# facebookresearch/iris

Measured on AMD Instinct MI355X. Metric: bake_shading throughput (shading samples/s: secondary rays traced and shaded), higher is better.
Workload: dtype f32; 1 GPU; bake_shading train-view sequence (15 views evenly spaced among 32 cameras on a circle, one view per step), 1920x1080, SPP=128 per lobe, lobes=[0, 1, 2, 3, 4, 5, 6] (0=diffuse,1-6=specular), synthetic room seed=1 1000990 triangles, SLF H=256, Philox uniforms; pixels_per_view=2073600

## Files before the change

### iris_amd/_lib.py

```python
import ctypes as C
import os

import torch

_HERE = os.path.dirname(os.path.abspath(__file__))
LIB_PATH = os.environ.get("IRIS_HIP_LIB") or os.path.join(_HERE, "libiris_hip.so")

BVH_DEFAULT, BVH4_F32, BVH4_Q8 = 0, 1, 3
BAKE_AUTO, BAKE_PIXEL_PER_WAVE, BAKE_TILE_SORTED = 0, 1, 2


class IrisError(RuntimeError):
    pass


class SceneInfo(C.Structure):
    _fields_ = [("n_vertices", C.c_int64), ("n_triangles", C.c_int64), ("layout", C.c_int32), ("n_nodes", C.c_int32),
                ("node_bytes", C.c_int32), ("tri_bytes", C.c_int32), ("depth", C.c_int32), ("n_leaf_records", C.c_int32),
                ("sah_cost", C.c_float), ("build_seconds", C.c_float)]


_P, _I64, _I32, _F, _D, _U64, _U32 = C.c_void_p, C.c_int64, C.c_int, C.c_float, C.c_double, C.c_uint64, C.c_uint32


# ... 143 lines not shown
    "iris_version": [],
}
_RESTYPE = {"iris_scene_destroy": None, "iris_slf_destroy": None, "iris_emitter_destroy": None,
            "iris_last_error": C.c_char_p, "iris_version": C.c_char_p, "iris_debug_build_flags": C.c_char_p, "iris_debug_source_hash": C.c_char_p, "iris_ngp_n_params": C.c_int64, "iris_ngp_destroy": None, "iris_bake_workspace_bytes": C.c_uint64, "iris_pt_compact_workspace_bytes": C.c_uint64, "iris_denoise_workspace_bytes": C.c_uint64,
            "iris_exr_zip_workspace_bytes": C.c_uint64, "iris_ngp_backward_workspace_bytes": C.c_uint64, "iris_crf_bwd_workspace_bytes": C.c_uint64,
            "iris_loss_photometric_workspace_bytes": C.c_uint64,
            "iris_png_row_bytes": C.c_int64, "iris_png_stream_bound": C.c_uint64, "iris_png_workspace_bytes": C.c_uint64, "iris_png_magma_table": None,
            "iris_jpeg_stream_bound": C.c_uint64, "iris_jpeg_workspace_bytes": C.c_uint64, "iris_jpeg_tables": None,
            "iris_image_metrics_workspace_bytes": C.c_uint64, "iris_uv_raster_workspace_bytes": C.c_uint64, "iris_atlas_density": C.c_double}

_lib = None


def lib():
    global _lib
    if _lib is None:
        if not os.path.exists(LIB_PATH):
            raise IrisError(f"{LIB_PATH} is missing: build it with `make -C iris_amd/csrc` or "
                            "`python -c 'import __graft_entry__ as g; g.build()'`. There is no CPU fallback.")
        l = C.CDLL(LIB_PATH)
        for name, argtypes in PROTOTYPES.items():
            fn = getattr(l, name)
            fn.argtypes = argtypes
            fn.restype = _RESTYPE.get(name, C.c_int)
        _lib = l
    return _lib


def source_hash():
    import hashlib
    h = hashlib.sha256()
    h.update(lib().iris_debug_build_flags())
    root = os.path.dirname(_HERE)
    files = [os.path.join("iris_amd", "csrc", f) for f in ("bvh_build.cpp", "bvh_build.h", "iris_bake.h", "iris_device.h", "iris_hip.hip", "iris_tile.h", "iris_trace.h")]
    files += [os.path.join("include", "iris_hip.h"), os.path.join("include", "iris_hip_debug.h")]
    for f in files:
        h.update(f.encode()); h.update(open(os.path.join(root, f), "rb").read())
    return h.hexdigest()[:16]


def device_index(device):
    device = torch.device(device)
    if device.type != "cuda":
        raise IrisError(f"{device}: the HIP path needs a GPU device (there is no CPU fallback)")
    return device.index if device.index is not None else torch.cuda.current_device()


class Native:

    def __init__(self, ptr=None, destroy=None, device=None, keys=()):
        self.ptr, self.destroy, self.device, self.keys = ptr, destroy, device, list(keys)

    def free(self):
        d = self.__dict__
        p, d["ptr"] = d.get("ptr"), None
        if p:
            d["destroy"](p)

    def __del__(self):
        try:
            self.free()
        except Exception:
            pass

    def __reduce__(self):
        return (Native, ())

# ... 93 lines not shown
```

### iris_amd/csrc/iris_bake.h

```cpp
#pragma once
#include "iris_tile.h"

namespace iris {

struct BakeArgs {
    SceneDev sc; EmitDev em; SlfDev slf;
    const float* pos; const float* nrm; const float* wo;
    const float* u2; const int32_t* pix_id;
    int64_t P; int spp; uint64_t seed; uint32_t stream_id; float rough;
    float* out0; float* out1; int64_t* tri_next;
    int64_t* src_next;
    unsigned long long* stats;
    uint32_t* stack_ovf;
    float4* scratch;
    unsigned int* tile_counter;
    int tile_px;
};

#ifndef IRIS_TILE_RAYS
#define IRIS_TILE_RAYS 5120
#endif
constexpr int kTileRays = IRIS_TILE_RAYS;

__device__ __forceinline__ void reduce_geometry(int spp, int& lpp, int& ppw, int& rounds) {
// ... 219 lines not shown
                    const f3 pn = hit_position(h, mk3(tx.x, ty.x, tz.x), mk3(tx.y, ty.y, tz.y), mk3(tx.z, ty.z, tz.z));
                    q = make_float4(pn.x, pn.y, pn.z, ow);
                }
                res[r] = q;
            } else
            res[r] = make_float4(h.u, h.v, __int_as_float(h.slot), 0.f);
            if (COUNT) n_rays++; }
        );

    const int n_groups = (np + ppw - 1) / ppw;
    IRIS_PHASE_BEGIN();
    for (int g = wave; g < n_groups; g += kBlock / 64) {
        const int pl = g * ppw + sub;
        const bool pvalid = pl < np;
        float a0x = 0.f, a0y = 0.f, a0z = 0.f, a1x = 0.f, a1y = 0.f, a1z = 0.f;
        if (resolve) {
            for (int rr = 0; rr < rounds; rr += 2) {
                const int s0 = rr * 64 + sl, s1 = s0 + 64;
                const bool ok0 = pvalid && s0 < spp, ok1 = pvalid && rr + 1 < rounds && s1 < spp;
                float4 q0 = make_float4(0.f, 0.f, 0.f, __int_as_float(-2)), q1 = q0;
                float2 w0 = make_float2(0.f, 0.f), w1 = w0;
                if (ok0) { q0 = res[pl * spp + s0]; if (SPEC) w0 = res_g[pl * spp + s0]; }
                if (ok1) { q1 = res[pl * spp + s1]; if (SPEC) w1 = res_g[pl * spp + s1]; }
                const int o0 = __float_as_int(q0.w), o1 = __float_as_int(q1.w);
                int j0 = -1, j1 = -1;
                if (o0 == -1) j0 = slf_index(a.slf, mk3(q0.x, q0.y, q0.z));
                if (o1 == -1) j1 = slf_index(a.slf, mk3(q1.x, q1.y, q1.z));
                float4 r0 = make_float4(0.f, 0.f, 0.f, 0.f), r1 = r0;
                if (o0 >= 0 || j0 >= 0) r0 = *(o0 >= 0 ? a.em.radiance + o0 : a.slf.radiance + j0);
                if (o1 >= 0 || j1 >= 0) r1 = *(o1 >= 0 ? a.em.radiance + o1 : a.slf.radiance + j1);
                if (ok0) {
                    const float z = o0 >= 0 ? -0.f : 0.f;
                    const f3 Le = mk3(z + r0.x, z + r0.y, z + r0.z);
                    if (a.src_next) a.src_next[(p0 + pl) * spp + s0] = o0 >= 0 ? -2 - o0 : j0;
                    if (SPEC) { a0x += Le.x * w0.y; a0y += Le.y * w0.y; a0z += Le.z * w0.y; a1x += Le.x * w0.x; a1y += Le.y * w0.x; a1z += Le.z * w0.x; }
                    else { a0x += Le.x; a0y += Le.y; a0z += Le.z; }
                }
                if (ok1) {
                    const float z = o1 >= 0 ? -0.f : 0.f;
                    const f3 Le = mk3(z + r1.x, z + r1.y, z + r1.z);
                    if (a.src_next) a.src_next[(p0 + pl) * spp + s1] = o1 >= 0 ? -2 - o1 : j1;
                    if (SPEC) { a0x += Le.x * w1.y; a0y += Le.y * w1.y; a0z += Le.z * w1.y; a1x += Le.x * w1.x; a1y += Le.y * w1.x; a1z += Le.z * w1.x; }
                    else { a0x += Le.x; a0y += Le.y; a0z += Le.z; }
                }
            }
        } else
        for (int rr = 0; rr < rounds; ++rr) {
            const int s = rr * 64 + sl;
            if (pvalid && s < spp) {
                const float4 qa = res[pl * spp + s];
                Hit h; h.u = qa.x; h.v = qa.y; h.slot = __float_as_int(qa.z); h.t = 0.f; h.id = 0;
                f3 pn = mk3(0.f, 0.f, 0.f);
                int64_t tri = -1;
                int ord_rec = -1;
                if (h.slot >= 0) {
                    const float4* tr = a.sc.tris + (int64_t)h.slot * 4;
                    const float4 tx = tr[0], ty = tr[1], tz = tr[2];
                    if (!a.em.emit_ord) ord_rec = __float_as_int(tr[3].x);
                    pn = hit_position(h, mk3(tx.x, ty.x, tz.x), mk3(tx.y, ty.y, tz.y), mk3(tx.z, ty.z, tz.z));
                    tri = __float_as_int(tx.w);
                }
                if (a.tri_next) a.tri_next[(p0 + pl) * spp + s] = tri;
                float epdf; bool vn; int src;
                const f3 Le = eval_emitter1(a.em, a.slf, pn, tri, true, 1.0f, 0.0f, epdf, vn, src, ord_rec);
                if (a.src_next) a.src_next[(p0 + pl) * spp + s] = src;
                if (SPEC) {
                    const float2 qb = res_g[pl * spp + s];
                    a0x += Le.x * qb.y; a0y += Le.y * qb.y; a0z += Le.z * qb.y;
                    a1x += Le.x * qb.x; a1y += Le.y * qb.x; a1z += Le.z * qb.x;
                } else { a0x += Le.x; a0y += Le.y; a0z += Le.z; }
            }
        }
        for (int m = 1; m < lpp; m <<= 1) {
            a0x += __shfl_xor(a0x, m); a0y += __shfl_xor(a0y, m); a0z += __shfl_xor(a0z, m);
// ... 100 lines not shown
```

### iris_amd/csrc/iris_device.h

```cpp
#pragma once
#include <hip/hip_runtime.h>
#include <stdint.h>

namespace iris {

struct f3 { float x, y, z; };
__device__ __forceinline__ f3 mk3(float x, float y, float z) { f3 r; r.x = x; r.y = y; r.z = z; return r; }
__device__ __forceinline__ f3 ld3(const float* p) { return mk3(p[0], p[1], p[2]); }
__device__ __forceinline__ void st3(float* p, f3 a) { p[0] = a.x; p[1] = a.y; p[2] = a.z; }
__device__ __forceinline__ f3 sub3(f3 a, f3 b) { return mk3(a.x - b.x, a.y - b.y, a.z - b.z); }

__device__ __forceinline__ f3 x_cross(f3 a, f3 b) {
    return mk3(fmaf(a.y, b.z, -(a.z * b.y)), fmaf(a.z, b.x, -(a.x * b.z)), fmaf(a.x, b.y, -(a.y * b.x)));
}
__device__ __forceinline__ float x_dot(f3 a, f3 b) { return fmaf(a.z, b.z, fmaf(a.y, b.y, a.x * b.x)); }

__device__ __forceinline__ float t_dot(f3 a, f3 b) { return (a.x * b.x + a.y * b.y) + a.z * b.z; }
__device__ __forceinline__ f3 t_normalize(f3 a) {
    float n = sqrtf((a.x * a.x + a.y * a.y) + a.z * a.z);
    n = fmaxf(n, 1e-12f);
    return mk3(a.x / n, a.y / n, a.z / n);
}
__device__ __forceinline__ f3 t_cross(f3 a, f3 b) {
    return mk3(a.y * b.z - a.z * b.y, a.z * b.x - a.x * b.z, a.x * b.y - a.y * b.x);
}
__device__ __forceinline__ float relu(float x) { return x > 0.f ? x : 0.f; }

constexpr float kPi = 3.14159265358979323846f;
constexpr float kTwoPi = 6.28318530717958647692f;
constexpr float kRayEps = 8.940696716308594e-05f;

__device__ __forceinline__ void normal_space(f3 n, f3& t, f3& b) {
    if (fabsf(n.x) <= 0.1f) t = t_normalize(mk3(0.f, -n.z, n.y));
    else                    t = t_normalize(mk3(n.z, 0.f, -n.x));
    b = t_cross(n, t);
// ... 104 lines not shown
    return r;
}

__device__ __forceinline__ void philox_u2(uint64_t seed, uint64_t idx, uint32_t stream, float& u0, float& u1) {
    uint32_t c0 = (uint32_t)idx, c1 = (uint32_t)(idx >> 32), c2 = stream, c3 = 0u;
    uint32_t k0 = (uint32_t)seed, k1 = (uint32_t)(seed >> 32);
#pragma unroll
    for (int r = 0; r < 10; ++r) {
        if (r) { k0 += 0x9E3779B9u; k1 += 0xBB67AE85u; }
        const uint64_t m0 = (uint64_t)0xD2511F53u * (uint64_t)c0, m1 = (uint64_t)0xCD9E8D57u * (uint64_t)c2;
        uint32_t h0 = (uint32_t)(m0 >> 32), l0 = (uint32_t)m0;
        uint32_t h1 = (uint32_t)(m1 >> 32), l1 = (uint32_t)m1;
        uint32_t n0 = h1 ^ c1 ^ k0, n2 = h0 ^ c3 ^ k1;
        c0 = n0; c1 = l1; c2 = n2; c3 = l0;
    }
    u0 = (float)(c0 >> 8) * 5.9604644775390625e-08f;
    u1 = (float)(c1 >> 8) * 5.9604644775390625e-08f;
}

__device__ __forceinline__ void philox4x32(uint64_t seed, uint64_t idx, uint32_t stream, uint32_t& o0, uint32_t& o1, uint32_t& o2, uint32_t& o3) {
    uint32_t c0 = (uint32_t)idx, c1 = (uint32_t)(idx >> 32), c2 = stream, c3 = 0u;
    uint32_t k0 = (uint32_t)seed, k1 = (uint32_t)(seed >> 32);
#pragma unroll
    for (int r = 0; r < 10; ++r) {
        if (r) { k0 += 0x9E3779B9u; k1 += 0xBB67AE85u; }
        const uint64_t m0 = (uint64_t)0xD2511F53u * (uint64_t)c0, m1 = (uint64_t)0xCD9E8D57u * (uint64_t)c2;
        const uint32_t n0 = (uint32_t)(m1 >> 32) ^ c1 ^ k0, n2 = (uint32_t)(m0 >> 32) ^ c3 ^ k1;
        c0 = n0; c1 = (uint32_t)m1; c2 = n2; c3 = (uint32_t)m0;
    }
    o0 = c0; o1 = c1; o2 = c2; o3 = c3;
}

struct SlfDev {
    const int32_t* inds;
    const float4* radiance;
    int H;
    float vmin, den;
};
struct EmitDev {
    const int32_t* emit_ord;
    const float4* radiance;
    const float* area;
    int64_t nf;
    float emitter_pdf;
};

__device__ __forceinline__ int voxel_coord(float p, const SlfDev& s) {
    float f = (p - s.vmin) / s.den * (float)s.H;
    int v = (int)f;
    if (!(f < 0x1p63f)) v = 0;
    return min(max(v, 0), s.H - 1);
}
__device__ __forceinline__ int slf_index(const SlfDev& s, f3 p) {
    int cx = voxel_coord(p.x, s), cy = voxel_coord(p.y, s), cz = voxel_coord(p.z, s);
    return s.inds[((int64_t)cz * s.H + cy) * s.H + cx];
}
__device__ __forceinline__ f3 slf_forward(const SlfDev& s, f3 p, int& j) {
    j = slf_index(s, p);
    if (j < 0) return mk3(0.f, 0.f, 0.f);
    float4 r = s.radiance[j];
    return mk3(r.x, r.y, r.z);
}
__device__ __forceinline__ f3 slf_forward(const SlfDev& s, f3 p) { int j; return slf_forward(s, p, j); }
__device__ __forceinline__ f3 eval_emitter1(const EmitDev& e, const SlfDev& s, f3 p, int64_t tri, bool has_rough,
                                            float rough, float trace_rough, float& emit_pdf, bool& valid_next, int& src, int ord_known = -1) {
    bool vis = tri != -1;
    f3 Le = mk3(0.f, 0.f, 0.f);
    emit_pdf = 0.f;
    int ord = -1;
    if (vis) ord = e.emit_ord ? e.emit_ord[tri < 0 ? tri + e.nf : tri] : ord_known;
    bool is_area = ord >= 0;
    src = -1;
    if (is_area) {
        src = -2 - ord;
        float4 r = e.radiance[ord];
        Le = mk3(r.x, r.y, r.z);
        emit_pdf = e.emitter_pdf / fmaxf(e.area[ord], 1e-12f);
    }
    valid_next = (!is_area) && vis;
    if (has_rough && (!is_area) && vis && rough > trace_rough) {
        f3 d = slf_forward(s, p, src);
        Le = mk3(Le.x + d.x, Le.y + d.y, Le.z + d.z);
        if ((d.x + d.y) + d.z > 0.f) valid_next = false;
    }
    return Le;
}
__device__ __forceinline__ f3 eval_emitter1(const EmitDev& e, const SlfDev& s, f3 p, int64_t tri, bool has_rough,
                                            float rough, float trace_rough, float& emit_pdf, bool& valid_next) {
    int src;
    return eval_emitter1(e, s, p, tri, has_rough, rough, trace_rough, emit_pdf, valid_next, src);
}

}
// ... 1 lines not shown
```

### iris_amd/csrc/iris_hip.hip

```cpp
#include <hip/hip_runtime.h>

#include <chrono>
#include <cmath>
#include <cstdio>
#include <cstring>
#include <atomic>
#include <cstdlib>
#include <memory>
#include <mutex>
#include <string>
#include <vector>

#include "../../include/iris_hip.h"
#include "../../include/iris_hip_debug.h"
#include "bvh_build.h"
#include "iris_device.h"
#include "iris_trace.h"
#include "iris_bake.h"
#include "iris_pt.h"
#include "iris_relight.h"
#include "iris_cache.h"
#include "iris_denoise.h"
#include "iris_metrics.h"
#include "iris_texture.h"
// ... 61 lines not shown
    else if (k == "tiles_per_block") g_opt_tiles_per_block = value;
    else if (k == "pt_tile_min") g_opt_pt_tile_min = value;
    else if (k == "joint_max_rays") g_opt_joint_max_rays = value;
    else if (k == "prop_bwd_targets") g_opt_prop_bwd_targets = value;
    else if (k == "prop_lds_members") g_opt_prop_lds_members = value;
    else if (k == "pool_combine") g_opt_pool_combine = value;
    else return fail(IRIS_ERR_ARG, "iris_debug_set: unknown option " + k);
    return IRIS_OK;
}
extern "C" IRIS_API const char* iris_version(void) { return "iris_hip 0.1 (gfx950)"; }
#ifndef IRIS_NO_FUSED_RECORDS
#define IRIS_NO_FUSED_RECORDS 0
#endif
#ifndef IRIS_BUILD_FLAGS
#define IRIS_BUILD_FLAGS "unknown"
#endif
extern "C" IRIS_API const char* iris_debug_build_flags(void) { return IRIS_BUILD_FLAGS; }
#ifndef IRIS_SOURCE_HASH
#define IRIS_SOURCE_HASH "unknown"
#endif
extern "C" IRIS_API const char* iris_debug_source_hash(void) { return IRIS_SOURCE_HASH; }

static std::atomic<uint64_t> g_scene_uid{1};
struct iris_scene {
    int device = 0;
    uint64_t uid = g_scene_uid.fetch_add(1);
    SceneDev dev{};
    DevBuf d_nodes, d_tris;
    iris_scene_info info{};
};
struct iris_slf {
    int device = 0;
    SlfDev dev{};
    DevBuf d_inds, d_rad;
    int64_t kv = 0;
    iris_slf(int device_, int64_t kv_) : device(device_), kv(kv_) {}
    void bind(int H, double voxel_min, double voxel_max) {
        dev.inds = (const int32_t*)d_inds.p; dev.radiance = (const float4*)d_rad.p; dev.H = H;
        dev.vmin = (float)voxel_min;
        dev.den = (float)(voxel_max - voxel_min);
    }
};
struct iris_emitter {
    int device = 0;
    EmitDev dev{};
    DevBuf d_ord, d_rad, d_area;
    DevBuf d_verts;
    DevBuf d_cdf;
    DevBuf d_ord2tri;
    EmitSampleDev sample{};
    bool can_sample = false;
    int64_t n_rad = 0, k = 0;
    struct Fused { uint64_t scene_uid; DevBuf d_tris; DevEvent ready; bool done; };
    mutable std::mutex fused_mu;
    mutable std::vector<Fused> fused;
    mutable std::vector<Fused> retired;
};

constexpr long long kJointMaxRays = 1 << 20;
static bool joint_launch(int64_t n_rays) { return n_rays <= (g_opt_joint_max_rays >= 0 ? g_opt_joint_max_rays : kJointMaxRays); }

template <int LAYOUT, bool JOINT = false> struct TraceTag { static constexpr int layout = LAYOUT; static constexpr bool joint = JOINT; };
template <class F> static void with_layout(const SceneDev& sc, F&& f) {
    if (sc.layout == kLayoutQ8) f(TraceTag<kLayoutQ8>{});
    else f(TraceTag<kLayoutF32>{});
}
template <class F> static void with_trace(const SceneDev& sc, int64_t n_rays, F&& f) {
    if (sc.layout == kLayoutQ8 && joint_launch(n_rays)) f(TraceTag<kLayoutQ8, true>{});
    else with_layout(sc, f);
}
template <bool SPEC, bool STATS, int LAYOUT> struct BakeTag { static constexpr bool spec = SPEC, stats = STATS; static constexpr int layout = LAYOUT; };
// ... 64 lines not shown
    auto s = std::make_unique<iris_scene>();
    s->device = device;
    if (s->d_nodes.alloc(nodes.size() * 4) != hipSuccess || s->d_tris.alloc(tris.size() * 4) != hipSuccess ||
        s->d_nodes.upload(nodes.data(), nodes.size() * 4) != hipSuccess || s->d_tris.upload(tris.data(), tris.size() * 4) != hipSuccess)
        return fail(IRIS_ERR_HIP, "iris_scene_create: device allocation / upload failed");
    s->dev.nodes = (const float4*)s->d_nodes.p;
    s->dev.tris = (const float4*)s->d_tris.p;
    s->dev.n_nodes = (int)nn;
    s->dev.n_tris = (int)nt;
    s->dev.layout = layout == IRIS_BVH4_Q8 ? kLayoutQ8 : kLayoutF32;
    s->dev.oct_stride = layout == IRIS_BVH4_Q8 ? (uint32_t)(nn * kNodeBytes) : 0u;
    s->dev.phase_min = kPhaseMin;
    if (g_opt_phase_min >= 0) s->dev.phase_min = (int)g_opt_phase_min;
    s->info.n_vertices = nv; s->info.n_triangles = nf; s->info.layout = layout; s->info.n_nodes = (int32_t)nn;
    s->info.node_bytes = (int)(layout == IRIS_BVH4_Q8 ? kNodeBytes : kNodeBytesF32); s->info.tri_bytes = (int)kLeafRecordBytes; s->info.depth = bvh.depth;
    s->info.sah_cost = bvh.sah_cost; s->info.n_leaf_records = (int32_t)nt;
    s->info.build_seconds = std::chrono::duration<float>(std::chrono::steady_clock::now() - t0).count();
    *out = s.release();
    return IRIS_OK;
    API_END
}
extern "C" IRIS_API void iris_scene_destroy(iris_scene* s) { delete s; }
extern "C" IRIS_API int iris_scene_get_info(const iris_scene* s, iris_scene_info* out) {
    if (!s || !out) return fail(IRIS_ERR_ARG, "iris_scene_get_info: null");
    *out = s->info;
    return IRIS_OK;
}

extern "C" IRIS_API int iris_slf_create(const int64_t* inds, int H, const float* radiance, int64_t kv, double voxel_min, double voxel_max,
                               int device, iris_slf** out) {
    API_BEGIN
    if (!out || !inds || H <= 0 || H > 1024 || kv < 0 || (kv > 0 && !radiance)) return fail(IRIS_ERR_ARG, "iris_slf_create: bad arguments");
    HIP_TRY(hipSetDevice(device));
    const size_t n = (size_t)H * H * H;
    std::vector<int32_t> i32(n);
    for (size_t i = 0; i < n; ++i) {
        int64_t v = inds[i];
        if (v < -1 || v >= kv) return fail(IRIS_ERR_ARG, "iris_slf_create: inds entry out of range");
        i32[i] = (int32_t)v;
    }
    std::vector<float> rad((size_t)std::max<int64_t>(kv, 1) * 4, 0.f);
    for (int64_t i = 0; i < kv; ++i) { rad[i * 4] = radiance[i * 3]; rad[i * 4 + 1] = radiance[i * 3 + 1]; rad[i * 4 + 2] = radiance[i * 3 + 2]; }
    auto s = std::make_unique<iris_slf>(device, kv);
    HIP_TRY(s->d_inds.alloc(n * 4));
    HIP_TRY(s->d_rad.alloc(rad.size() * 4));
    HIP_TRY(s->d_inds.upload(i32.data(), n * 4));
    HIP_TRY(s->d_rad.upload(rad.data(), rad.size() * 4));
    s->bind(H, voxel_min, voxel_max);
    *out = s.release();
    return IRIS_OK;
    API_END
}
__global__ void slf_inds_narrow_kernel(const int64_t* __restrict__ src, int32_t* __restrict__ dst, int64_t n, int64_t kv, int* __restrict__ bad) {
    for (int64_t i = blockIdx.x * (int64_t)blockDim.x + threadIdx.x; i < n; i += (int64_t)gridDim.x * blockDim.x) {
        const int64_t v = src[i];
        if (v < -1 || v >= kv) *bad = 1;
        dst[i] = (int32_t)v;
    }
}
__global__ void pad_rows_kernel(const float* __restrict__ src, float4* __restrict__ dst, int64_t n) {
    for (int64_t i = blockIdx.x * (int64_t)blockDim.x + threadIdx.x; i < n; i += (int64_t)gridDim.x * blockDim.x)
        dst[i] = make_float4(src[i * 3], src[i * 3 + 1], src[i * 3 + 2], 0.f);
}
extern "C" IRIS_API int iris_slf_create_dev(const int64_t* inds_dev, int H, const float* radiance_dev, int64_t kv, double voxel_min, double voxel_max,
                                   int device, iris_slf** out, iris_stream_t stream) {
    API_BEGIN
    if (!out || !inds_dev || H <= 0 || H > 1024 || kv < 0 || (kv > 0 && !radiance_dev)) return fail(IRIS_ERR_ARG, "iris_slf_create_dev: bad arguments");
    HIP_TRY(hipSetDevice(device));
    const size_t n = (size_t)H * H * H;
    auto s = std::make_unique<iris_slf>(device, kv);
    DevBuf d_bad;
    if (s->d_inds.alloc(n * 4) != hipSuccess || s->d_rad.alloc((size_t)std::max<int64_t>(kv, 1) * 16) != hipSuccess || d_bad.alloc(4) != hipSuccess)
        return fail(IRIS_ERR_HIP, "iris_slf_create_dev: out of device memory");
    hipStream_t st = (hipStream_t)stream;
    (void)hipMemsetAsync(d_bad.p, 0, 4, st);
    (void)hipMemsetAsync(s->d_rad.p, 0, (size_t)std::max<int64_t>(kv, 1) * 16, st);
    hipLaunchKernelGGL(slf_inds_narrow_kernel, dim3(grid_for((int64_t)n, 256, 8192)), dim3(256), 0, st, inds_dev, (int32_t*)s->d_inds.p, (int64_t)n, kv, (int*)d_bad.p);
    if (kv > 0) hipLaunchKernelGGL(pad_rows_kernel, dim3(grid_for(kv, 256, 1024)), dim3(256), 0, st, radiance_dev, (float4*)s->d_rad.p, kv);
    int bad = 0;
    if (hipMemcpyAsync(&bad, d_bad.p, 4, hipMemcpyDeviceToHost, st) != hipSuccess || hipStreamSynchronize(st) != hipSuccess) return fail(IRIS_ERR_HIP, "iris_slf_create_dev: HIP error");
    if (bad) return fail(IRIS_ERR_ARG, "iris_slf_create_dev: inds entry out of range");
    s->bind(H, voxel_min, voxel_max);
    *out = s.release();
    return IRIS_OK;
    API_END
}
extern "C" IRIS_API void iris_slf_destroy(iris_slf* s) { delete s; }

struct iris_ngp {
    int device = 0;
    NgpLevels lv{};
    DevBuf d_grid;
    DevBuf d_w;
    DevBuf d_feat;
    float vmin = 0.f, den = 1.f;
    uint64_t n_entries = 0;
    mutable std::mutex mu;
    mutable DevEvent last_use;
    mutable hipStream_t last_stream = nullptr;
    mutable bool used = false;
};
constexpr int kNgpChunk = 1 << 20;
static uint64_t ngp_levels(NgpLevels& lv) {
    const float log2_scale = (float)log2((double)1.3f);
    uint64_t off = 0;
    for (int l = 0; l < kNgpLevels; ++l) {
        const float scale = (float)exp2((double)((float)l * log2_scale)) * 16.f - 1.0f;
        const uint32_t res = (uint32_t)ceilf(scale) + 1u;
        uint64_t n = (uint64_t)res * res * res;
        n = std::min<uint64_t>(n, 0xFFFFFFFFull / 2);
        n = (n + 7) / 8 * 8;
        n = std::min<uint64_t>(n, 1ull << 19);
        lv.scale[l] = scale; lv.res[l] = res; lv.size[l] = (uint32_t)n; lv.offset[l] = (uint32_t)off;
        off += n;
// ... 200 lines not shown
    e->device = device; e->n_rad = n_rad; e->k = k;
    HIP_TRY(e->d_ord.alloc(ord.size() * 4));
    HIP_TRY(e->d_rad.alloc(rad.size() * 4));
    HIP_TRY(e->d_area.alloc((size_t)std::max<int64_t>(k, 1) * 4));
    HIP_TRY(e->d_ord.upload(ord.data(), ord.size() * 4));
    HIP_TRY(e->d_rad.upload(rad.data(), rad.size() * 4));
    if (k > 0) HIP_TRY(e->d_area.upload(area, (size_t)k * 4));
    e->dev.emit_ord = (const int32_t*)e->d_ord.p; e->dev.radiance = (const float4*)e->d_rad.p; e->dev.area = (const float*)e->d_area.p;
    e->dev.nf = nf;
    float kf = (float)k; if (kf < 1e-12f) kf = 1e-12f;
    e->dev.emitter_pdf = 1.0f / kf;
    if (verts && cdf && k > 0) {
        std::vector<int32_t> o2t((size_t)k);
        for (int64_t i = 0; i < nf; ++i) if (ord[(size_t)i] >= 0) o2t[(size_t)ord[(size_t)i]] = (int32_t)i;
        HIP_TRY(e->d_verts.alloc((size_t)k * 36));
        HIP_TRY(e->d_cdf.alloc((size_t)k * 4));
        HIP_TRY(e->d_ord2tri.alloc((size_t)k * 4));
        HIP_TRY(e->d_verts.upload(verts, (size_t)k * 36));
        HIP_TRY(e->d_cdf.upload(cdf, (size_t)k * 4));
        HIP_TRY(e->d_ord2tri.upload(o2t.data(), (size_t)k * 4));
        e->sample.cdf = (const float*)e->d_cdf.p; e->sample.verts = (const float*)e->d_verts.p; e->sample.area = (const float*)e->d_area.p;
        e->sample.ord2tri = (const int32_t*)e->d_ord2tri.p; e->sample.k = k; e->sample.emitter_pdf = e->dev.emitter_pdf;
        e->can_sample = true;
    }
    *out = e.release();
    return IRIS_OK;
    API_END
}
extern "C" IRIS_API void iris_emitter_destroy(iris_emitter* e) { delete e; }

extern "C" IRIS_API int iris_slf_set_radiance(iris_slf* s, const float* radiance_dev, int64_t kv, iris_stream_t stream) {
    if (!s || kv != s->kv || (kv > 0 && !radiance_dev)) return fail(IRIS_ERR_ARG, "iris_slf_set_radiance: bad arguments");
    if (kv == 0) return IRIS_OK;
    return launch1d(pad_rows_kernel, kv, 1024, stream, radiance_dev, (float4*)s->d_rad.p, kv);
}
extern "C" IRIS_API int iris_emitter_set_radiance(iris_emitter* e, const float* radiance_dev, int64_t n_rad, iris_stream_t stream) {
    if (!e || !radiance_dev || n_rad != e->n_rad) return fail(IRIS_ERR_ARG, "iris_emitter_set_radiance: bad arguments");
    return launch1d(pad_rows_kernel, n_rad, 1024, stream, radiance_dev, (float4*)e->d_rad.p, n_rad);
}

struct RaygenArgs { float K[9]; float c2w[12]; float focal; int H, W, ray_diff, synthetic; };

__global__ void raygen_kernel(RaygenArgs a, float* __restrict__ rays_o, float* __restrict__ rays_d, float* __restrict__ dxdu,
                              float* __restrict__ dydv) {
    const int64_t n = (int64_t)a.H * a.W;
    for (int64_t i = blockIdx.x * (int64_t)blockDim.x + threadIdx.x; i < n; i += (int64_t)gridDim.x * blockDim.x) {
        const int y = (int)(i / a.W), x = (int)(i - (int64_t)y * a.W);
        const PixelRay r = raygen_pixel(a.K, a.c2w, a.focal, a.H, a.W, a.ray_diff, a.synthetic, x, y);
        st3(rays_o + i * 3, r.o);
        st3(rays_d + i * 3, r.d);
        if (a.ray_diff) {
            st3(dxdu + i * 3, r.dxdu);
            st3(dydv + i * 3, r.dydv);
        }
    }
}
static int raygen_launch(RaygenArgs a, float* o, float* d, float* dx, float* dy, iris_stream_t stream) {
    if (a.H <= 0 || a.W <= 0 || !o || !d || (a.ray_diff && (!dx || !dy))) return fail(IRIS_ERR_ARG, "iris_raygen: bad arguments");
    return launch1d(raygen_kernel, (int64_t)a.H * a.W, 4096, stream, a, o, d, dx, dy);
}
extern "C" IRIS_API int iris_raygen_real(const float K[9], const float c2w[12], int H, int W, int ray_diff, float* rays_o, float* rays_d,
                                float* dxdu, float* dydv, iris_stream_t stream) {
    if (!K || !c2w) return fail(IRIS_ERR_ARG, "iris_raygen_real: null K/c2w");
    RaygenArgs a{};
    std::memcpy(a.K, K, 36); std::memcpy(a.c2w, c2w, 48);
    a.H = H; a.W = W; a.ray_diff = ray_diff; a.synthetic = 0; a.focal = 1.f;
    return raygen_launch(a, rays_o, rays_d, dxdu, dydv, stream);
// ... 90 lines not shown
__global__ void sample_specular_kernel(const float* __restrict__ u2, const float* __restrict__ wo, const float* __restrict__ normal,
                                       float rough_all, const float* __restrict__ rough_each, int64_t B, float* __restrict__ wi, float* __restrict__ pdf,
                                       float* __restrict__ w0, float* __restrict__ w1) {
    for (int64_t i = blockIdx.x * (int64_t)blockDim.x + threadIdx.x; i < B; i += (int64_t)gridDim.x * blockDim.x) {
        f3 n = ld3(normal + i * 3), o = ld3(wo + i * 3), t, b;
        const float rough = rough_each ? rough_each[i] : rough_all;
        normal_space(n, t, b);
        f3 d = specular_sampler(u2[i * 2], u2[i * 2 + 1], rough, o, n, t, b);
        SpecW w = specular_weights(d, o, n, rough, pdf != nullptr);
        st3(wi + i * 3, d);
        if (pdf) pdf[i] = w.pdf;
        if (w0) w0[i] = w.g0;
        if (w1) w1[i] = w.g1;
    }
}
extern "C" IRIS_API int iris_sample_specular(const float* u2, const float* wo, const float* normal, float roughness, int64_t B, float* wi,
                                    float* pdf, float* w0, float* w1, iris_stream_t stream) {
    if (B < 0 || (B > 0 && (!u2 || !wo || !normal || !wi))) return fail(IRIS_ERR_ARG, "iris_sample_specular: bad arguments");
    if (B == 0) return IRIS_OK;
    return launch1d(sample_specular_kernel, B, 8192, stream, u2, wo, normal, roughness,
                       (const float*)nullptr, B, wi, pdf, w0, w1);
}
extern "C" IRIS_API int iris_sample_specular_v(const float* u2, const float* wo, const float* normal, const float* roughness, int64_t B, float* wi,
                                      float* pdf, float* w0, float* w1, iris_stream_t stream) {
    if (B < 0 || (B > 0 && (!u2 || !wo || !normal || !roughness || !wi))) return fail(IRIS_ERR_ARG, "iris_sample_specular_v: bad arguments");
    if (B == 0) return IRIS_OK;
    return launch1d(sample_specular_kernel, B, 8192, stream, u2, wo, normal, 0.f, roughness, B,
                       wi, pdf, w0, w1);
}

__global__ void slf_lookup_kernel(SlfDev s, const float* __restrict__ x, int64_t B, int64_t* __restrict__ idx, float* __restrict__ rgb) {
    for (int64_t i = blockIdx.x * (int64_t)blockDim.x + threadIdx.x; i < B; i += (int64_t)gridDim.x * blockDim.x) {
        f3 p = ld3(x + i * 3);
        int j = slf_index(s, p);
        if (idx) idx[i] = j;
        if (rgb) {
            f3 r = mk3(0.f, 0.f, 0.f);
            if (j >= 0) { float4 q = s.radiance[j]; r = mk3(q.x, q.y, q.z); }
            st3(rgb + i * 3, r);
        }
    }
}
extern "C" IRIS_API int iris_slf_lookup(const iris_slf* s, const float* x, int64_t B, int64_t* idx, float* rgb, iris_stream_t stream) {
    if (!s || B < 0 || (B > 0 && !x)) return fail(IRIS_ERR_ARG, "iris_slf_lookup: bad arguments");
    if (B == 0) return IRIS_OK;
    return launch1d(slf_lookup_kernel, B, 8192, stream, s->dev, x, B, idx, rgb);
}

__global__ void eval_emitter_kernel(EmitDev e, SlfDev s, const float* __restrict__ pos, const int64_t* __restrict__ tri,
                                    const float* __restrict__ rough, float trace_rough, int64_t B, float* __restrict__ Le,
                                    float* __restrict__ emit_pdf, uint8_t* __restrict__ valid_next) {
    for (int64_t i = blockIdx.x * (int64_t)blockDim.x + threadIdx.x; i < B; i += (int64_t)gridDim.x * blockDim.x) {
        float pdf; bool vn;
        f3 l = eval_emitter1(e, s, ld3(pos + i * 3), tri[i], rough != nullptr, rough ? rough[i] : 0.f, trace_rough, pdf, vn);
        st3(Le + i * 3, l);
        if (emit_pdf) emit_pdf[i] = pdf;
        if (valid_next) valid_next[i] = vn ? 1 : 0;
    }
}
extern "C" IRIS_API int iris_eval_emitter(const iris_emitter* e, const iris_slf* s, const float* position, const int64_t* triangle_idx,
                                 const float* roughness, float trace_roughness, int64_t B, float* Le, float* emit_pdf,
                                 uint8_t* valid_next, iris_stream_t stream) {
    const bool slf_unreachable = !roughness || (std::isinf(trace_roughness) && trace_roughness > 0.f);
    if (!e || (!s && !slf_unreachable) || B < 0 || (B > 0 && (!position || !triangle_idx || !Le))) return fail(IRIS_ERR_ARG, "iris_eval_emitter: bad arguments");
    if (B == 0) return IRIS_OK;
    return launch1d(eval_emitter_kernel, B, 8192, stream, e->dev, s ? s->dev : SlfDev{}, position,
                       triangle_idx, roughness, trace_roughness, B, Le, emit_pdf, valid_next);
}

__global__ void lerp_specular_kernel(const float* __restrict__ spec, const float* __restrict__ rough, int64_t B, int R, float* __restrict__ out) {
    for (int64_t i = blockIdx.x * (int64_t)blockDim.x + threadIdx.x; i < B; i += (int64_t)gridDim.x * blockDim.x) {
        float r = (rough[i] - 0.02f) / (float)(1.0 - 0.02) * (float)(R - 1);
        int r1 = min(max((int)ceilf(r), 0), R - 1), r0 = min(max((int)floorf(r), 0), R - 1);
// ... 1495 lines not shown
```

### iris_amd/csrc/iris_prebake.h

```cpp
#pragma once
#include <hip/hip_runtime.h>
#include <stdint.h>

#include "iris_batch.h"
#include "iris_crf.h"
#include "iris_device.h"
#include "iris_prop.h"
#include "iris_trace.h"

namespace iris {

__device__ __forceinline__ void pool_hist(float* __restrict__ hist, const SlfDev& s, f3 p) {
    const int cx = voxel_coord(p.x, s), cy = voxel_coord(p.y, s), cz = voxel_coord(p.z, s);
    atomicAdd(hist + ((int64_t)cz * s.H + cy) * s.H + cx, 1.0f);
}
__device__ __forceinline__ void pool_voxel(const SlfDev& s, f3 p, f3 rgb, float* __restrict__ acc, unsigned long long* __restrict__ count) {
    const int j = slf_index(s, p);
    if (j < 0) return;
    atomicAdd(acc + (int64_t)j * 3, rgb.x); atomicAdd(acc + (int64_t)j * 3 + 1, rgb.y); atomicAdd(acc + (int64_t)j * 3 + 2, rgb.z);
    atomicAdd(count + j, 1ull);
}
__device__ __forceinline__ void pool_triangle(int64_t j, int64_t F, f3 rgb, float* __restrict__ out, float* __restrict__ count) {
    if (j < 0 || j >= F) return;
    atomicAdd(out + j * 3, rgb.x); atomicAdd(out + j * 3 + 1, rgb.y); atomicAdd(out + j * 3 + 2, rgb.z);
    if (count) atomicAdd(count + j, 1.0f);
}

__device__ __forceinline__ void atomic_min_float(float* addr, float x) {
    x = x + 0.0f;
    if (x >= 0.f) atomicMin((int*)addr, __float_as_int(x));
    else atomicMax((unsigned int*)addr, __float_as_uint(x));
}
__device__ __forceinline__ void atomic_max_float(float* addr, float x) {
    x = x + 0.0f;
    if (x >= 0.f) atomicMax((int*)addr, __float_as_int(x));
    else atomicMin((unsigned int*)addr, __float_as_uint(x));
}

template <class Body>
__device__ __forceinline__ void for_each_destination(long long key, Body&& body) {
    unsigned long long todo = __ballot(key >= 0);
    while (todo) {
        const int lead = __ffsll(todo) - 1;
        const bool mine = key == __shfl(key, lead);
        const unsigned long long lanes = __ballot(mine);
        body(mine, lanes, (int)(threadIdx.x & 63) == lead);
        todo &= ~lanes;
    }
}
template <class C>
// ... 59 lines not shown
                    rgb = mk3(s_lut[u[0]], s_lut[256 + u[1]], s_lut[512 + u[2]]);
                } else {
                    rgb = ld3((const float*)a.rgb + i * 3);
                    if (crf) {
                        rgb.x = crf_value(a.crf.table, crf_segment_uniform(a.crf.grid, a.crf.n, crf_clip(rgb.x)));
                        rgb.y = crf_value(a.crf.table + a.crf.n, crf_segment_uniform(a.crf.grid, a.crf.n, crf_clip(rgb.y)));
                        rgb.z = crf_value(a.crf.table + 2 * a.crf.n, crf_segment_uniform(a.crf.grid, a.crf.n, crf_clip(rgb.z)));
                    }
                }
                if (crf) {
                    const float e = crf_exposure(a.crf, i);
                    rgb = mk3(rgb.x / e, rgb.y / e, rgb.z / e);
                }
            }
        }
        if (!a.combine) {
            if (hit) {
                if (a.hist) pool_hist(a.hist, a.hist_grid, p);
                if (want_rgb && a.has_slf) pool_voxel(a.slf, p, rgb, a.slf_acc, a.slf_count);
                if (want_rgb && a.tri_sum) pool_triangle(h.id, a.n_tri, rgb, a.tri_sum, a.tri_count);
            }
            continue;
        }
        if (a.hist) {
            long long key = -1;
            if (hit) {
                const SlfDev& s = a.hist_grid;
                key = ((long long)voxel_coord(p.z, s) * s.H + voxel_coord(p.y, s)) * s.H + voxel_coord(p.x, s);
            }
            for_each_destination(key, [&](bool, unsigned long long lanes, bool leader) {
                if (leader) atomicAdd(a.hist + key, (float)__popcll(lanes));
            });
        }
        if (want_rgb && a.has_slf) pool_rows_combined(hit ? (long long)slf_index(a.slf, p) : -1, rgb, a.slf_acc, a.slf_count);
        if (want_rgb && a.tri_sum) pool_rows_combined(hit && h.id < a.n_tri ? (long long)h.id : -1, rgb, a.tri_sum, a.tri_count);
    }
    if (a.bounds) {
#pragma unroll
        for (int m = 32; m > 0; m >>= 1) {
            lo = fminf(lo, __shfl_xor(lo, m));
            hi = fmaxf(hi, __shfl_xor(hi, m));
        }
        if ((threadIdx.x & 63) == 0) { s_lo[threadIdx.x >> 6] = lo; s_hi[threadIdx.x >> 6] = hi; }
        __syncthreads();
        if (threadIdx.x == 0) {
#pragma unroll
            for (int w = 1; w < kBlock / 64; ++w) { lo = fminf(lo, s_lo[w]); hi = fmaxf(hi, s_hi[w]); }
            if (lo <= hi) {
                atomic_min_float(a.bounds, lo);
                atomic_max_float(a.bounds + 1, hi);
            }
        }
    }
}

}
```

Baseline: 10380 Mrays/s.

## Replace dense SLF voxel index grid with rank/select bitmap table

Replaces the dense H^3 int32 voxel-to-row index array with a compact bitmap plus prefix-count table (8 bytes per 32 voxels), and reorders radiance rows by rank with the original row id stored in the w lane. Lookups become a popcount over a small cached record instead of a random 4-byte read from a 64 MB table, which is meant to cut cache misses in the bake resolve path. It adds GPU scan kernels for building the table and extra indirection through the stored row id wherever the original index is needed.

```diff
diff --git a/iris_amd/_lib.py b/iris_amd/_lib.py
--- a/iris_amd/_lib.py
+++ b/iris_amd/_lib.py
@@ -199,7 +199,7 @@
     h = hashlib.sha256()
     h.update(lib().iris_debug_build_flags())
     root = os.path.dirname(_HERE)
-    files = [os.path.join("iris_amd", "csrc", f) for f in ("bvh_build.cpp", "bvh_build.h", "iris_bake.h", "iris_device.h", "iris_hip.hip", "iris_tile.h", "iris_trace.h")]
+    files = [os.path.join("iris_amd", "csrc", f) for f in ("bvh_build.cpp", "bvh_build.h", "iris_bake.h", "iris_device.h", "iris_hip.hip", "iris_slf_rank.h", "iris_tile.h", "iris_trace.h")]
     files += [os.path.join("include", "iris_hip.h"), os.path.join("include", "iris_hip_debug.h")]
     for f in files:
         h.update(f.encode()); h.update(open(os.path.join(root, f), "rb").read())
diff --git a/iris_amd/csrc/iris_bake.h b/iris_amd/csrc/iris_bake.h
--- a/iris_amd/csrc/iris_bake.h
+++ b/iris_amd/csrc/iris_bake.h
@@ -275,14 +275,14 @@
                 if (ok0) {
                     const float z = o0 >= 0 ? -0.f : 0.f;
                     const f3 Le = mk3(z + r0.x, z + r0.y, z + r0.z);
-                    if (a.src_next) a.src_next[(p0 + pl) * spp + s0] = o0 >= 0 ? -2 - o0 : j0;
+                    if (a.src_next) a.src_next[(p0 + pl) * spp + s0] = o0 >= 0 ? -2 - o0 : j0 >= 0 ? __float_as_int(r0.w) : -1;
                     if (SPEC) { a0x += Le.x * w0.y; a0y += Le.y * w0.y; a0z += Le.z * w0.y; a1x += Le.x * w0.x; a1y += Le.y * w0.x; a1z += Le.z * w0.x; }
                     else { a0x += Le.x; a0y += Le.y; a0z += Le.z; }
                 }
                 if (ok1) {
                     const float z = o1 >= 0 ? -0.f : 0.f;
                     const f3 Le = mk3(z + r1.x, z + r1.y, z + r1.z);
-                    if (a.src_next) a.src_next[(p0 + pl) * spp + s1] = o1 >= 0 ? -2 - o1 : j1;
+                    if (a.src_next) a.src_next[(p0 + pl) * spp + s1] = o1 >= 0 ? -2 - o1 : j1 >= 0 ? __float_as_int(r1.w) : -1;
                     if (SPEC) { a0x += Le.x * w1.y; a0y += Le.y * w1.y; a0z += Le.z * w1.y; a1x += Le.x * w1.x; a1y += Le.y * w1.x; a1z += Le.z * w1.x; }
                     else { a0x += Le.x; a0y += Le.y; a0z += Le.z; }
                 }
diff --git a/iris_amd/csrc/iris_device.h b/iris_amd/csrc/iris_device.h
--- a/iris_amd/csrc/iris_device.h
+++ b/iris_amd/csrc/iris_device.h
@@ -1,6 +1,8 @@
 #pragma once
 #include <hip/hip_runtime.h>
 #include <stdint.h>
+
+#include "iris_slf_rank.h"
 
 namespace iris {
 
@@ -171,11 +173,12 @@
 }
 
 struct SlfDev {
-    const int32_t* inds;
+    const SlfRankRecord* rank;
     const float4* radiance;
     int H;
     float vmin, den;
 };
+static_assert(sizeof(SlfDev) == 32, "SlfDev travels by value in BakeArgs / ViewArgs: the bake kernels' scalar-register budget has no room for it to grow");
 struct EmitDev {
     const int32_t* emit_ord;
     const float4* radiance;
@@ -192,12 +195,17 @@
 }
 __device__ __forceinline__ int slf_index(const SlfDev& s, f3 p) {
     int cx = voxel_coord(p.x, s), cy = voxel_coord(p.y, s), cz = voxel_coord(p.z, s);
-    return s.inds[((int64_t)cz * s.H + cy) * s.H + cx];
+    return slf_rank_lookup(s.rank, s.H, cx, cy, cz);
+}
+__device__ __forceinline__ int slf_row(const SlfDev& s, f3 p) {
+    const int j = slf_index(s, p);
+    return j < 0 ? -1 : __float_as_int(s.radiance[j].w);
 }
 __device__ __forceinline__ f3 slf_forward(const SlfDev& s, f3 p, int& j) {
     j = slf_index(s, p);
     if (j < 0) return mk3(0.f, 0.f, 0.f);
     float4 r = s.radiance[j];
+    j = __float_as_int(r.w);
     return mk3(r.x, r.y, r.z);
 }
 __device__ __forceinline__ f3 slf_forward(const SlfDev& s, f3 p) { int j; return slf_forward(s, p, j); }
diff --git a/iris_amd/csrc/iris_hip.hip b/iris_amd/csrc/iris_hip.hip
--- a/iris_amd/csrc/iris_hip.hip
+++ b/iris_amd/csrc/iris_hip.hip
@@ -117,11 +117,13 @@
 struct iris_slf {
     int device = 0;
     SlfDev dev{};
-    DevBuf d_inds, d_rad;
+    DevBuf d_rank, d_rad;
+    DevBuf d_row_of_rank;
     int64_t kv = 0;
+    int64_t n_rows = 0;
     iris_slf(int device_, int64_t kv_) : device(device_), kv(kv_) {}
     void bind(int H, double voxel_min, double voxel_max) {
-        dev.inds = (const int32_t*)d_inds.p; dev.radiance = (const float4*)d_rad.p; dev.H = H;
+        dev.rank = (const SlfRankRecord*)d_rank.p; dev.radiance = (const float4*)d_rad.p; dev.H = H;
         dev.vmin = (float)voxel_min;
         dev.den = (float)(voxel_max - voxel_min);
     }
@@ -252,30 +254,92 @@
     API_BEGIN
     if (!out || !inds || H <= 0 || H > 1024 || kv < 0 || (kv > 0 && !radiance)) return fail(IRIS_ERR_ARG, "iris_slf_create: bad arguments");
     HIP_TRY(hipSetDevice(device));
-    const size_t n = (size_t)H * H * H;
-    std::vector<int32_t> i32(n);
-    for (size_t i = 0; i < n; ++i) {
-        int64_t v = inds[i];
-        if (v < -1 || v >= kv) return fail(IRIS_ERR_ARG, "iris_slf_create: inds entry out of range");
-        i32[i] = (int32_t)v;
-    }
-    std::vector<float> rad((size_t)std::max<int64_t>(kv, 1) * 4, 0.f);
-    for (int64_t i = 0; i < kv; ++i) { rad[i * 4] = radiance[i * 3]; rad[i * 4 + 1] = radiance[i * 3 + 1]; rad[i * 4 + 2] = radiance[i * 3 + 2]; }
+    SlfRank rk;
+    if (!slf_rank_build(inds, H, kv, rk)) return fail(IRIS_ERR_ARG, "iris_slf_create: inds entry out of range");
+    std::vector<float> rad((size_t)std::max<int64_t>(rk.n_rows, 1) * 4, 0.f);
+    slf_rank_pack_rows(radiance, rk.identity() ? nullptr : rk.row_of_rank.data(), rk.n_rows, rad.data());
     auto s = std::make_unique<iris_slf>(device, kv);
-    HIP_TRY(s->d_inds.alloc(n * 4));
+    s->n_rows = rk.n_rows;
+    HIP_TRY(s->d_rank.alloc(slf_rank_bytes(H)));
     HIP_TRY(s->d_rad.alloc(rad.size() * 4));
-    HIP_TRY(s->d_inds.upload(i32.data(), n * 4));
+    HIP_TRY(s->d_rank.upload(rk.table.data(), slf_rank_bytes(H)));
     HIP_TRY(s->d_rad.upload(rad.data(), rad.size() * 4));
+    if (!rk.identity()) {
+        HIP_TRY(s->d_row_of_rank.alloc(rk.row_of_rank.size() * 4));
+        HIP_TRY(s->d_row_of_rank.upload(rk.row_of_rank.data(), rk.row_of_rank.size() * 4));
+    }
     s->bind(H, voxel_min, voxel_max);
     *out = s.release();
     return IRIS_OK;
     API_END
 }
-__global__ void slf_inds_narrow_kernel(const int64_t* __restrict__ src, int32_t* __restrict__ dst, int64_t n, int64_t kv, int* __restrict__ bad) {
+constexpr uint32_t kRankScanChunk = 1024;
+__global__ void slf_rank_bits_kernel(const int64_t* __restrict__ inds, SlfRankRecord* __restrict__ tab, uint32_t n, uint32_t nw, int64_t kv, int* __restrict__ flags) {
+    const uint32_t lane = threadIdx.x & 63u, ng = (n + 63u) >> 6;
+    for (uint32_t g = blockIdx.x * 4u + (threadIdx.x >> 6); g < ng; g += gridDim.x * 4u) {
+        const uint32_t v = g * 64u + lane;
+        int64_t r = -1;
+        if (v < n) r = inds[v];
+        if (r < -1 || r >= kv) { flags[0] = 1; r = -1; }
+        const uint64_t b = __ballot(r >= 0);
+        if (lane == 0) {
+            const uint32_t lo = (uint32_t)b, hi = (uint32_t)(b >> 32), w = g * 2u;
+            tab[w] = SlfRankRecord{lo, (uint32_t)__popc(lo)};
+            if (w + 1u < nw) tab[w + 1u] = SlfRankRecord{hi, (uint32_t)__popc(hi)};
+        }
+    }
+}
+__device__ __forceinline__ uint32_t block_scan_256(uint32_t x, uint32_t* sh) {
+    sh[threadIdx.x] = x;
+    __syncthreads();
+    for (uint32_t off = 1; off < 256u; off <<= 1) {
+        const uint32_t y = threadIdx.x >= off ? sh[threadIdx.x - off] : 0u;
+        __syncthreads();
+        sh[threadIdx.x] += y;
+        __syncthreads();
+    }
+    return sh[threadIdx.x];
+}
+__global__ void slf_rank_scan_chunk_kernel(SlfRankRecord* __restrict__ tab, uint32_t nw, uint32_t* __restrict__ chunk_sum) {
+    __shared__ uint32_t sh[256];
+    const uint32_t base = blockIdx.x * kRankScanChunk + threadIdx.x * 4u;
+    uint32_t c[4], t = 0;
+    for (int k = 0; k < 4; ++k) { c[k] = base + k < nw ? tab[base + k].count : 0u; t += c[k]; }
+    uint32_t run = block_scan_256(t, sh) - t;
+    for (int k = 0; k < 4; ++k) { if (base + k < nw) tab[base + k].count = run; run += c[k]; }
+    if (threadIdx.x == 255) chunk_sum[blockIdx.x] = sh[255];
+}
+__global__ void slf_rank_scan_sums_kernel(uint32_t* __restrict__ chunk_sum, uint32_t nb, int* __restrict__ flags) {
+    __shared__ uint32_t sh[256];
+    const uint32_t per = (nb + 255u) / 256u, lo = threadIdx.x * per, hi = min(lo + per, nb);
+    uint32_t t = 0;
+    for (uint32_t i = lo; i < hi; ++i) t += chunk_sum[i];
+    uint32_t run = block_scan_256(t, sh) - t;
+    for (uint32_t i = lo; i < hi; ++i) { const uint32_t x = chunk_sum[i]; chunk_sum[i] = run; run += x; }
+    if (threadIdx.x == 255) flags[1] = (int)sh[255];
+}
+__global__ void slf_rank_scan_add_kernel(SlfRankRecord* __restrict__ tab, uint32_t nw, const uint32_t* __restrict__ chunk_sum) {
+    for (uint32_t w = blockIdx.x * blockDim.x + threadIdx.x; w < nw; w += gridDim.x * blockDim.x) tab[w].count += chunk_sum[w / kRankScanChunk];
+}
+__global__ void slf_rank_identity_kernel(const int64_t* __restrict__ inds, const SlfRankRecord* __restrict__ tab, uint32_t n, int* __restrict__ flags) {
+    for (uint32_t v = blockIdx.x * blockDim.x + threadIdx.x; v < n; v += gridDim.x * blockDim.x) {
+        const int64_t r = inds[v];
+        if (r >= 0 && r != (int64_t)slf_rank_lookup_linear(tab, v)) flags[2] = 1;
+    }
+}
+__global__ void slf_rank_rows_kernel(const int64_t* __restrict__ inds, const SlfRankRecord* __restrict__ tab, uint32_t n, const float* __restrict__ radiance, float4* __restrict__ rad, int32_t* __restrict__ row_of_rank) {
+    for (uint32_t v = blockIdx.x * blockDim.x + threadIdx.x; v < n; v += gridDim.x * blockDim.x) {
+        const int64_t r = inds[v];
+        if (r < 0) continue;
+        const uint32_t k = (uint32_t)slf_rank_lookup_linear(tab, v);
+        rad[k] = make_float4(radiance[r * 3], radiance[r * 3 + 1], radiance[r * 3 + 2], __int_as_float((int)r));
+        if (row_of_rank) row_of_rank[k] = (int32_t)r;
+    }
+}
+__global__ void slf_pad_rows_kernel(const float* __restrict__ src, const int32_t* __restrict__ row_of_rank, float4* __restrict__ dst, int64_t n) {
     for (int64_t i = blockIdx.x * (int64_t)blockDim.x + threadIdx.x; i < n; i += (int64_t)gridDim.x * blockDim.x) {
-        const int64_t v = src[i];
-        if (v < -1 || v >= kv) *bad = 1;
-        dst[i] = (int32_t)v;
+        const int64_t r = row_of_rank ? row_of_rank[i] : i;
+        dst[i] = make_float4(src[r * 3], src[r * 3 + 1], src[r * 3 + 2], __int_as_float((int)r));
     }
 }
 __global__ void pad_rows_kernel(const float* __restrict__ src, float4* __restrict__ dst, int64_t n) {
@@ -287,19 +351,35 @@
     API_BEGIN
     if (!out || !inds_dev || H <= 0 || H > 1024 || kv < 0 || (kv > 0 && !radiance_dev)) return fail(IRIS_ERR_ARG, "iris_slf_create_dev: bad arguments");
     HIP_TRY(hipSetDevice(device));
-    const size_t n = (size_t)H * H * H;
+    const uint32_t n = (uint32_t)H * (uint32_t)H * (uint32_t)H, nw = slf_rank_records(H), nb = (nw + kRankScanChunk - 1) / kRankScanChunk;
     auto s = std::make_unique<iris_slf>(device, kv);
-    DevBuf d_bad;
-    if (s->d_inds.alloc(n * 4) != hipSuccess || s->d_rad.alloc((size_t)std::max<int64_t>(kv, 1) * 16) != hipSuccess || d_bad.alloc(4) != hipSuccess)
+    DevBuf d_flags, d_sums;
+    if (s->d_rank.alloc(slf_rank_bytes(H)) != hipSuccess || d_flags.alloc(3 * sizeof(int)) != hipSuccess || d_sums.alloc((size_t)nb * 4) != hipSuccess)
         return fail(IRIS_ERR_HIP, "iris_slf_create_dev: out of device memory");
     hipStream_t st = (hipStream_t)stream;
-    (void)hipMemsetAsync(d_bad.p, 0, 4, st);
-    (void)hipMemsetAsync(s->d_rad.p, 0, (size_t)std::max<int64_t>(kv, 1) * 16, st);
-    hipLaunchKernelGGL(slf_inds_narrow_kernel, dim3(grid_for((int64_t)n, 256, 8192)), dim3(256), 0, st, inds_dev, (int32_t*)s->d_inds.p, (int64_t)n, kv, (int*)d_bad.p);
-    if (kv > 0) hipLaunchKernelGGL(pad_rows_kernel, dim3(grid_for(kv, 256, 1024)), dim3(256), 0, st, radiance_dev, (float4*)s->d_rad.p, kv);
-    int bad = 0;
-    if (hipMemcpyAsync(&bad, d_bad.p, 4, hipMemcpyDeviceToHost, st) != hipSuccess || hipStreamSynchronize(st) != hipSuccess) return fail(IRIS_ERR_HIP, "iris_slf_create_dev: HIP error");
-    if (bad) return fail(IRIS_ERR_ARG, "iris_slf_create_dev: inds entry out of range");
+    SlfRankRecord* tab = (SlfRankRecord*)s->d_rank.p;
+    HIP_TRY(hipMemsetAsync(d_flags.p, 0, 3 * sizeof(int), st));
+    hipLaunchKernelGGL(slf_rank_bits_kernel, dim3(grid_for(((int64_t)n + 63) / 64, 4, 8192)), dim3(256), 0, st, inds_dev, tab, n, nw, kv, (int*)d_flags.p);
+    hipLaunchKernelGGL(slf_rank_scan_chunk_kernel, dim3(nb), dim3(256), 0, st, tab, nw, (uint32_t*)d_sums.p);
+    hipLaunchKernelGGL(slf_rank_scan_sums_kernel, dim3(1), dim3(256), 0, st, (uint32_t*)d_sums.p, nb, (int*)d_flags.p);
+    hipLaunchKernelGGL(slf_rank_scan_add_kernel, dim3(grid_for((int64_t)nw, 256, 8192)), dim3(256), 0, st, tab, nw, (const uint32_t*)d_sums.p);
+    hipLaunchKernelGGL(slf_rank_identity_kernel, dim3(grid_for((int64_t)n, 256, 8192)), dim3(256), 0, st, inds_dev, (const SlfRankRecord*)tab, n, (int*)d_flags.p);
+    HIP_TRY(hipGetLastError());
+    int flags[3] = {0, 0, 0};
+    if (hipMemcpyAsync(flags, d_flags.p, sizeof(flags), hipMemcpyDeviceToHost, st) != hipSuccess || hipStreamSynchronize(st) != hipSuccess) return fail(IRIS_ERR_HIP, "iris_slf_create_dev: HIP error");
+    if (flags[0]) return fail(IRIS_ERR_ARG, "iris_slf_create_dev: inds entry out of range");
+    s->n_rows = flags[1];
+    const bool identity = !flags[2] && s->n_rows == kv;
+    const size_t rad_bytes = (size_t)std::max<int64_t>(s->n_rows, 1) * 16;
+    if (s->d_rad.alloc(rad_bytes) != hipSuccess || (!identity && s->n_rows > 0 && s->d_row_of_rank.alloc((size_t)s->n_rows * 4) != hipSuccess))
+        return fail(IRIS_ERR_HIP, "iris_slf_create_dev: out of device memory");
+    HIP_TRY(hipMemsetAsync(s->d_rad.p, 0, rad_bytes, st));
+    if (s->n_rows > 0) {
+        hipLaunchKernelGGL(slf_rank_rows_kernel, dim3(grid_for((int64_t)n, 256, 8192)), dim3(256), 0, st, inds_dev, (const SlfRankRecord*)tab, n,
+                           radiance_dev, (float4*)s->d_rad.p, (int32_t*)s->d_row_of_rank.p);
+        HIP_TRY(hipGetLastError());
+        HIP_TRY(hipStreamSynchronize(st));
+    }
     s->bind(H, voxel_min, voxel_max);
     *out = s.release();
     return IRIS_OK;
@@ -566,7 +646,7 @@
 extern "C" IRIS_API int iris_slf_set_radiance(iris_slf* s, const float* radiance_dev, int64_t kv, iris_stream_t stream) {
     if (!s || kv != s->kv || (kv > 0 && !radiance_dev)) return fail(IRIS_ERR_ARG, "iris_slf_set_radiance: bad arguments");
     if (kv == 0) return IRIS_OK;
-    return launch1d(pad_rows_kernel, kv, 1024, stream, radiance_dev, (float4*)s->d_rad.p, kv);
+    return launch1d(slf_pad_rows_kernel, s->n_rows, 1024, stream, radiance_dev, (const int32_t*)s->d_row_of_rank.p, (float4*)s->d_rad.p, s->n_rows);
 }
 extern "C" IRIS_API int iris_emitter_set_radiance(iris_emitter* e, const float* radiance_dev, int64_t n_rad, iris_stream_t stream) {
     if (!e || !radiance_dev || n_rad != e->n_rad) return fail(IRIS_ERR_ARG, "iris_emitter_set_radiance: bad arguments");
@@ -723,13 +803,11 @@
 __global__ void slf_lookup_kernel(SlfDev s, const float* __restrict__ x, int64_t B, int64_t* __restrict__ idx, float* __restrict__ rgb) {
     for (int64_t i = blockIdx.x * (int64_t)blockDim.x + threadIdx.x; i < B; i += (int64_t)gridDim.x * blockDim.x) {
         f3 p = ld3(x + i * 3);
-        int j = slf_index(s, p);
+        int j;
+        f3 r = mk3(0.f, 0.f, 0.f);
+        if (rgb) r = slf_forward(s, p, j); else j = slf_row(s, p);
         if (idx) idx[i] = j;
-        if (rgb) {
-            f3 r = mk3(0.f, 0.f, 0.f);
-            if (j >= 0) { float4 q = s.radiance[j]; r = mk3(q.x, q.y, q.z); }
-            st3(rgb + i * 3, r);
-        }
+        if (rgb) st3(rgb + i * 3, r);
     }
 }
 extern "C" IRIS_API int iris_slf_lookup(const iris_slf* s, const float* x, int64_t B, int64_t* idx, float* rgb, iris_stream_t stream) {
diff --git a/iris_amd/csrc/iris_prebake.h b/iris_amd/csrc/iris_prebake.h
--- a/iris_amd/csrc/iris_prebake.h
+++ b/iris_amd/csrc/iris_prebake.h
@@ -15,7 +15,7 @@
     atomicAdd(hist + ((int64_t)cz * s.H + cy) * s.H + cx, 1.0f);
 }
 __device__ __forceinline__ void pool_voxel(const SlfDev& s, f3 p, f3 rgb, float* __restrict__ acc, unsigned long long* __restrict__ count) {
-    const int j = slf_index(s, p);
+    const int j = slf_row(s, p);
     if (j < 0) return;
     atomicAdd(acc + (int64_t)j * 3, rgb.x); atomicAdd(acc + (int64_t)j * 3 + 1, rgb.y); atomicAdd(acc + (int64_t)j * 3 + 2, rgb.z);
     atomicAdd(count + j, 1ull);
@@ -141,7 +141,7 @@
                 if (leader) atomicAdd(a.hist + key, (float)__popcll(lanes));
             });
         }
-        if (want_rgb && a.has_slf) pool_rows_combined(hit ? (long long)slf_index(a.slf, p) : -1, rgb, a.slf_acc, a.slf_count);
+        if (want_rgb && a.has_slf) pool_rows_combined(hit ? (long long)slf_row(a.slf, p) : -1, rgb, a.slf_acc, a.slf_count);
         if (want_rgb && a.tri_sum) pool_rows_combined(hit && h.id < a.n_tri ? (long long)h.id : -1, rgb, a.tri_sum, a.tri_count);
     }
     if (a.bounds) {
diff --git a/iris_amd/csrc/iris_slf_rank.h b/iris_amd/csrc/iris_slf_rank.h
--- /dev/null
+++ b/iris_amd/csrc/iris_slf_rank.h
@@ -0,0 +1,72 @@
+#pragma once
+#include <cstdint>
+#include <cstring>
+#include <vector>
+
+#if defined(__HIPCC__)
+#define IRIS_RANK_HD __host__ __device__ __forceinline__
+#else
+#define IRIS_RANK_HD inline
+#endif
+
+namespace iris {
+
+struct alignas(8) SlfRankRecord { uint32_t bits, count; };
+
+IRIS_RANK_HD uint32_t slf_rank_records(int H) { return ((uint32_t)H * (uint32_t)H * (uint32_t)H + 31u) >> 5; }
+IRIS_RANK_HD size_t slf_rank_bytes(int H) { return (size_t)slf_rank_records(H) * sizeof(SlfRankRecord); }
+
+IRIS_RANK_HD int slf_rank_lookup_linear(const SlfRankRecord* table, uint32_t v) {
+    const SlfRankRecord rec = table[v >> 5];
+    const uint32_t b = v & 31u;
+    const int rank = (int)(rec.count + (uint32_t)__builtin_popcount(rec.bits & ((1u << b) - 1u)));
+    return ((rec.bits >> b) & 1u) ? rank : -1;
+}
+IRIS_RANK_HD int slf_rank_lookup(const SlfRankRecord* table, int H, int cx, int cy, int cz) {
+#if defined(__HIP_DEVICE_COMPILE__)
+    return slf_rank_lookup_linear(table, __umul24(__umul24((uint32_t)cz, (uint32_t)H) + (uint32_t)cy, (uint32_t)H) + (uint32_t)cx);
+#else
+    return slf_rank_lookup_linear(table, ((uint32_t)cz * (uint32_t)H + (uint32_t)cy) * (uint32_t)H + (uint32_t)cx);
+#endif
+}
+
+struct SlfRank {
+    int H = 0;
+    std::vector<SlfRankRecord> table;
+    int64_t n_rows = 0;
+    std::vector<int32_t> row_of_rank;
+    bool identity() const { return row_of_rank.empty(); }
+};
+inline bool slf_rank_build(const int64_t* inds, int H, int64_t kv, SlfRank& out) {
+    const size_t n = (size_t)H * H * H;
+    out.H = H;
+    out.table.assign(slf_rank_records(H), SlfRankRecord{0u, 0u});
+    out.row_of_rank.clear();
+    bool ident = true;
+    uint32_t rank = 0;
+    for (size_t w = 0; w < out.table.size(); ++w) {
+        out.table[w].count = rank;
+        const size_t end = n - w * 32 < 32 ? n - w * 32 : 32;
+        for (size_t b = 0; b < end; ++b) {
+            const int64_t r = inds[w * 32 + b];
+            if (r < -1 || r >= kv) return false;
+            if (r < 0) continue;
+            out.table[w].bits |= 1u << b;
+            ident = ident && r == (int64_t)rank;
+            out.row_of_rank.push_back((int32_t)r);
+            ++rank;
+        }
+    }
+    out.n_rows = (int64_t)rank;
+    if (ident && out.n_rows == kv) { out.row_of_rank.clear(); out.row_of_rank.shrink_to_fit(); }
+    return true;
+}
+inline void slf_rank_pack_rows(const float* radiance, const int32_t* row_of_rank, int64_t n_rows, float* out4) {
+    for (int64_t i = 0; i < n_rows; ++i) {
+        const int32_t r = row_of_rank ? row_of_rank[i] : (int32_t)i;
+        out4[i * 4] = radiance[(int64_t)r * 3]; out4[i * 4 + 1] = radiance[(int64_t)r * 3 + 1]; out4[i * 4 + 2] = radiance[(int64_t)r * 3 + 2];
+        memcpy(out4 + i * 4 + 3, &r, 4);
+    }
+}
+
+}
```

Measured after the change: 10400 Mrays/s (median of 6 runs). Within noise of the previous version (+0.2%).
